# hanquansanren/DvD

Hardware: NVIDIA B200
Metric: dewarped docs/sec (sampling+unwarp) (higher is better)
Workload: dtype bf16x3 (split 16-bit operand pairs, 3 tcgen05 passes per k-step - 2 in the decoder q|k|v GEMMs and the pyramid convs -, fp32 accumulate: fp32-accurate)

## Files before the change

### dvd_b200/_lib.py

```python
from __future__ import annotations

import ctypes as C
import os

_HERE = os.path.dirname(os.path.abspath(__file__))
LIB_PATH = os.environ.get("DVD_LIB", os.path.join(_HERE, "libdvd_b200.so"))

PREC_FP32 = 0
PREC_BF16 = 1
PREC_BF16X3 = 2
TABLE_ROW = 384 + 2304 + 3072

_vp = C.c_void_p


class Mat(C.Structure):
    _fields_ = [("f32", _vp), ("bf16", _vp), ("bf16_lo", _vp), ("n", C.c_int32), ("k", C.c_int32)]


class DecLayer(C.Structure):
    _fields_ = [("n1_w", _vp), ("n1_b", _vp), ("qkv", Mat), ("fc", Mat), ("n2_w", _vp), ("n2_b", _vp),
                ("conv1", Mat), ("bn1_scale", _vp), ("bn1_shift", _vp), ("dw_w", _vp), ("bn2_scale", _vp),
                ("bn2_shift", _vp), ("conv2", Mat), ("bn3_scale", _vp), ("bn3_shift", _vp),
                ("qkv_ln", Mat), ("qkv_colsum", _vp), ("qkv_cvec", _vp), ("conv1_ln", Mat), ("conv1_colsum", _vp), ("conv1_cvec", _vp)]


class Weights(C.Structure):
    _fields_ = [("pos", _vp), ("pyr", Mat * 7), ("pyr_b", _vp * 7), ("emb", Mat * 5), ("emb_b", _vp * 5),
                ("t_mlp0", Mat), ("t_mlp2", Mat), ("t_mlp0_b", _vp), ("t_mlp2_b", _vp),
                ("blk_ada", Mat), ("blk_ada_b", _vp), ("xattn_in", Mat), ("xattn_in_b", _vp),
                ("xattn_out", Mat), ("xattn_out_b", _vp), ("blk_qkv", Mat), ("blk_qkv_b", _vp),
                ("blk_proj", Mat), ("blk_proj_b", _vp), ("blk_fc1", Mat), ("blk_fc1_b", _vp),
                ("blk_fc2", Mat), ("blk_fc2_b", _vp), ("dec_hpe", _vp), ("dec_wpe", _vp),
                ("h_scale0", Mat), ("h_scale2", Mat), ("w_scale0", Mat), ("w_scale2", Mat),
                ("h_scale0_b", _vp), ("h_scale2_b", _vp), ("w_scale0_b", _vp), ("w_scale2_b", _vp),
                ("dec", DecLayer * 6), ("dec_ln_w", _vp), ("dec_ln_b", _vp), ("fin", Mat), ("fin_b", _vp),
                ("fin_ada", Mat), ("fin_ada_b", _vp), ("pyr_h", Mat * 7)]


class UnwarpDoc(C.Structure):
    _fields_ = [("photo", _vp), ("out", _vp), ("H", C.c_int32), ("W", C.c_int32)]


_i, _f, _sz = C.c_int, C.c_float, C.c_size_t
_WP = C.POINTER(Weights)
_FP = C.POINTER(C.c_float)
SIGNATURES = {
    "dvd_version": (_i, []),
    "dvd_last_error": (C.c_char_p, []),
    "dvd_check_device": (_i, []),
    "dvd_unwarp_f32": (_i, [_vp, _vp, _vp, _i, _i, _i, _i, _i, _i, _f, _vp]),
    "dvd_unwarp_u8": (_i, [_vp, _vp, _vp, _i, _i, _i, _i, _i, _i, _f, _vp]),
    "dvd_unwarp_f32_u8": (_i, [_vp, _vp, _vp, _i, _i, _i, _i, _i, _i, _f, _vp]),
    "dvd_unwarp_table_bytes": (_sz, [_i]),
    "dvd_unwarp_u8_plan": (_i, [C.POINTER(UnwarpDoc), _i, _i, _i, _i, _f, _vp, _sz, C.POINTER(C.c_longlong)]),
    "dvd_unwarp_u8_mixed": (_i, [_vp, _i, _vp, _vp]),
    "dvd_grid_sample_f32": (_i, [_vp, _vp, _vp, _i, _i, _i, _i, _i, _i, _vp]),
    "dvd_fullres_grid_f32": (_i, [_vp, _vp, _i, _i, _i, _i, _i, _f, _vp]),
    "dvd_workspace_bytes": (_sz, [_i, _i, _i]),
    "dvd_tables_init": (_i, [_WP, _FP, _i, _vp, _vp]),
    "dvd_static_forward": (_i, [_WP, _vp, _sz, _i, _i, _i, _vp, _vp, _vp, _vp, _vp]),
    "dvd_denoise_step": (_i, [_WP, _vp, _sz, _i, _i, _i, _vp, _vp, _vp, _i, _vp, _f, _f, _vp, _vp, _vp]),
    "dvd_hyp_mean_clamp": (_i, [_vp, _vp, _i, _i, _vp]),
    "dvd_sample": (_i, [_WP, _vp, _sz, _i, _i, _i, _vp, _vp, _vp, _FP, _FP, _FP, _i, _vp, _vp, _vp]),
    "dvd_workspace_feat": (_vp, [_vp, _i, _i, _i]),
    "dvd_workspace_tensor": (_vp, [_vp, _i, _i, _i, C.c_char_p, C.POINTER(C.c_longlong)]),
    "dvd_test_gemm": (_i, [_vp, _vp, _vp, _vp, _i, _i, _i, _i, _vp, _sz, _vp]),
    "dvd_test_attention": (_i, [_vp, _vp, _vp, _vp, _i, _i, _i, _i, _f, _i, _vp, _sz, _vp]),
    "dvd_gemm_bf16": (_i, [_vp, _vp, _i, _vp, _vp, _i, _vp, _vp, _vp, _i, _i, _i, _vp]),
    "dvd_gemm_tune": (_i, [_vp, _vp, _i, _vp, _vp, _i, _vp, _vp, _vp, _i, _vp, _vp, _vp, _vp, _i, _i, _i, _vp]),
    "dvd_debug_stop_after": (_i, [_i]),
    "dvd_profile_begin": (_i, []),
    "dvd_profile_end": (_i, [C.POINTER(C.c_double), C.POINTER(C.c_double), C.POINTER(C.c_longlong), C.POINTER(C.c_double)]),
    "dvd_launch_count": (C.c_longlong, [_i]),
}

_lib = None


def lib() -> C.CDLL:
    global _lib
    if _lib is None:
        if not os.path.exists(LIB_PATH):
            raise RuntimeError(f"{LIB_PATH} not found: the CUDA extension has not been built "
                               "(run `python -m dvd_b200.build`). dvd_b200 has no CPU fallback.")
        l = C.CDLL(LIB_PATH)
        for name, (res, args) in SIGNATURES.items():
            fn = getattr(l, name)
            fn.restype = res
            fn.argtypes = args
        _lib = l
    return _lib


def check(rc: int, what: str = ""):
    if rc != 0:
        msg = lib().dvd_last_error().decode(errors="replace")
        raise RuntimeError(f"libdvd_b200 {what} failed (code {rc}): {msg}")


def ptr(t):
    return None if t is None else _vp(t.data_ptr())


def stream_ptr():
    import torch
    return _vp(torch.cuda.current_stream().cuda_stream)
```

### dvd_b200/csrc/api.cu

```cuda
#include <stdarg.h>
#include <string.h>
#include <stdlib.h>
#include "gemm_simt.cuh"
#include "gemm_tc.cuh"
#include "misc.cuh"

namespace dvd {

static thread_local char g_err[512] = "";
static thread_local long long g_launches = 0;

void set_error(const char* fmt, ...) {
  va_list ap;
  va_start(ap, fmt);
  vsnprintf(g_err, sizeof(g_err), fmt, ap);
  va_end(ap);
}
int cuda_fail(cudaError_t e, const char* what) {
  set_error("CUDA error %d (%s) at %s", (int)e, cudaGetErrorString(e), what);
  return (int)e;
}
void count_launch(int n) { g_launches += n; }
bool pdl_enabled(int kind) {
  static int mask = -1;
// ... 18 lines not shown
extern "C" const char* dvd_last_error(void) { return g_err; }
extern "C" long long dvd_launch_count(int reset) {
  long long v = g_launches;
  if (reset) g_launches = 0;
  return v;
}
extern "C" int dvd_check_device(void) {
  int dev = 0;
  DVD_CUDA(cudaGetDevice(&dev));
  cudaDeviceProp p;
  DVD_CUDA(cudaGetDeviceProperties(&p, dev));
  if (p.major != 10) {
    set_error("device %d is sm_%d%d; libdvd_b200 is built for sm_100a only", dev, p.major, p.minor);
    return DVD_E_ARCH;
  }
  return 0;
}

extern "C" int dvd_test_gemm(const float* A, const float* W, const float* bias, float* C, int M, int N, int K, int precision,
                             void* scratch, size_t scratch_bytes, void* stream) {
  cudaStream_t st = (cudaStream_t)stream;
  DVD_REQUIRE(A && W && C, "test_gemm: null");
  Epilogue e; e.bias = bias; e.out = C; e.ldc = N;
  if (precision == DVD_PREC_FP32) {
    GemmParams p = linear_params(A, K, W, M, N, K);
    p.e = e;
    return gemm_f32(p, A_DIRECT, B_NK, 1, st);
  }
  const bool a16 = precision == 3;
  const bool x3 = precision == DVD_PREC_BF16X3 || a16;
  auto al = [](size_t b) { return (b + 255) & ~size_t(255); };
  const size_t a_b = al((size_t)M * K * 2), w_b = al((size_t)N * K * 2);
  const size_t ops = (x3 ? 2 : 1) * (a_b + w_b);
  DVD_REQUIRE(scratch && scratch_bytes >= ops, "test_gemm: scratch needs %zu bytes", ops);
  char* base = (char*)scratch;
  TcMat a, w;
  a.hi = (__nv_bfloat16*)base; w.hi = (__nv_bfloat16*)(base + a_b); a.ld = K; w.ld = K;
  int rc;
  if (x3) {
    a.lo = (__nv_bfloat16*)(base + a_b + w_b); w.lo = (__nv_bfloat16*)(base + 2 * a_b + w_b);
    if (a16) { rc = f32_to_f16(A, (void*)a.hi, (long long)M * K, st); a.lo = nullptr; a.f16 = true; }
    else rc = f32_split_bf16(A, (__nv_bfloat16*)a.hi, (__nv_bfloat16*)a.lo, (long long)M * K, st);
    if (rc) return rc;
    rc = a16 ? f32_split_f16(W, (void*)w.hi, (void*)w.lo, (long long)N * K, st)
             : f32_split_bf16(W, (__nv_bfloat16*)w.hi, (__nv_bfloat16*)w.lo, (long long)N * K, st);
    if (rc) return rc;
  } else {
    rc = f32_to_bf16(A, (__nv_bfloat16*)a.hi, (long long)M * K, st); if (rc) return rc;
    rc = f32_to_bf16(W, (__nv_bfloat16*)w.hi, (long long)N * K, st); if (rc) return rc;
  }
  return gemm_tc(a, w, M, N, K, e, st);
}

extern "C" int dvd_test_attention(const float* q, const float* k, const float* v, float* o, int batch, int heads, int T, int d,
                                  float scale, int precision, void* scratch, size_t scratch_bytes, void* stream) {
  cudaStream_t st = (cudaStream_t)stream;
  DVD_REQUIRE(q && k && v && o && scratch, "test_attention: null");
  const int ld = heads * d;
  if (precision == DVD_PREC_FP32) {
    size_t per = (size_t)heads * T * T;
    DVD_REQUIRE(scratch_bytes >= per * batch * 4, "test_attention: scratch needs %zu bytes", per * batch * 4);
    float* S = (float*)scratch;
    GemmParams p;
    p.A = q; p.lda = ld; p.sAn = (long long)T * ld; p.sAh = d;
    p.B = k; p.ldb = ld; p.sBn = (long long)T * ld; p.sBh = d;
    p.M = T; p.N = T; p.K = d; p.heads = heads; p.alpha = scale;
    p.e.out = S; p.e.ldc = T; p.sCn = (long long)per; p.sCh = (long long)T * T;
    int rc = gemm_f32(p, A_DIRECT, B_NK, batch * heads, st); if (rc) return rc;
    rc = softmax_rows(S, (long long)batch * heads * T, T, st); if (rc) return rc;
    GemmParams g;
    g.A = S; g.lda = T; g.sAn = (long long)per; g.sAh = (long long)T * T;
    g.B = v; g.ldb = ld; g.sBn = (long long)T * ld; g.sBh = d;
    g.M = T; g.N = d; g.K = T; g.heads = heads;
    g.e.out = o; g.e.ldc = ld; g.sCn = (long long)T * ld; g.sCh = d;
    return gemm_f32(g, A_DIRECT, B_KN, batch * heads, st);
  }
  const bool x3 = precision == DVD_PREC_BF16X3;
  size_t n = (size_t)batch * T * ld;
  DVD_REQUIRE(scratch_bytes >= n * 2 * 6, "test_attention: scratch needs %zu bytes", n * 12);
  __nv_bfloat16* q16 = (__nv_bfloat16*)scratch; __nv_bfloat16* k16 = q16 + n; __nv_bfloat16* v16 = k16 + n; __nv_bfloat16* o16 = v16 + n;
  __nv_bfloat16* vt16 = o16 + n; __nv_bfloat16* olo = vt16 + n;
  int rc;
  if (x3) {
    rc = f32_to_f16(q, q16, n, st); if (rc) return rc;
    rc = f32_to_f16(k, k16, n, st); if (rc) return rc;
    rc = f32_to_f16(v, v16, n, st); if (rc) return rc;
  } else {
    rc = f32_to_bf16(q, q16, n, st); if (rc) return rc;
    rc = f32_to_bf16(k, k16, n, st); if (rc) return rc;
    rc = f32_to_bf16(v, v16, n, st); if (rc) return rc;
  }
  rc = transpose_v16(v16, ld, vt16, batch, T, ld, st); if (rc) return rc;
  rc = attention_tc(q16, ld, k16, ld, vt16, o16, x3 ? olo : nullptr, ld, batch, heads, T, d, scale, 1, x3 ? 1 : 0, st); if (rc) return rc;
  return pair_to_f32(o16, x3 ? olo : nullptr, o, n, st);
}

extern "C" int dvd_gemm_bf16(const void* A16, const void* A16_lo, int lda, const void* W16, const void* W16_lo, int ldw, const float* bias,
                             void* out16, float* out32, int M, int N, int K, void* stream) {
  Epilogue e; e.bias = bias; e.out_bf16 = (__nv_bfloat16*)out16; e.ldc_bf16 = N; e.out = out32; e.ldc = N;
  TcMat a, w;
  a.hi = (const __nv_bfloat16*)A16; a.lo = (const __nv_bfloat16*)A16_lo; a.ld = lda;
  a.f16 = !A16_lo && W16_lo;
  w.hi = (const __nv_bfloat16*)W16; w.lo = (const __nv_bfloat16*)W16_lo; w.ld = ldw;
  return gemm_tc(a, w, M, N, K, e, (cudaStream_t)stream);
}

// ... 13 lines not shown
```

### dvd_b200/csrc/misc.cu

```cuda
#include "misc.cuh"
#include "tc_epilogue.cuh"
#include <algorithm>

namespace dvd {

template <int NV>
__global__ void __launch_bounds__(256) k_layernorm(const float* __restrict__ in, int ldin, float* __restrict__ out, int ldo,
                                                   __nv_bfloat16* __restrict__ out16, __nv_bfloat16* __restrict__ out16_lo, int ldo16,
                                                   int rows, float eps, const float* __restrict__ w, const float* __restrict__ b,
                                                   const float* __restrict__ msh, const float* __restrict__ msc) {
  pdl_trigger();
  pdl_wait();
  const int row = blockIdx.x * 8 + (threadIdx.x >> 5), lane = threadIdx.x & 31;
  if (row >= rows) return;
  constexpr int C = 128 * NV;
  const float4* x4 = reinterpret_cast<const float4*>(in + (size_t)row * ldin);
  float4 v[NV];
  float s = 0.f;
#pragma unroll
  for (int i = 0; i < NV; ++i) { v[i] = __ldg(x4 + lane + 32 * i); s += (v[i].x + v[i].y) + (v[i].z + v[i].w); }
  const float mean = warp_sum(s) * (1.0f / C);
  float q = 0.f;
#pragma unroll
  for (int i = 0; i < NV; ++i) {
// ... 510 lines not shown
  float s1 = 0.f, s2 = 0.f;
#pragma unroll
  for (int i = 0; i < 12; ++i) {
    const int c = lane + 32 * i;
    float4 x = xr[c];
    const float4 a = __ldg(hs + (size_t)n * C4 + c), b = __ldg(ws + (size_t)n * C4 + c);
    const float4 hp = __ldg(hpe + (size_t)(tok >> 5) * C4 + c), wp = __ldg(wpe + (size_t)(tok & 31) * C4 + c);
    x.x = (x.x + a.x * hp.x) + b.x * wp.x; x.y = (x.y + a.y * hp.y) + b.y * wp.y;
    x.z = (x.z + a.z * hp.z) + b.z * wp.z; x.w = (x.w + a.w * hp.w) + b.w * wp.w;
    xr[c] = x;
    *reinterpret_cast<uint2*>(x16 + ((size_t)row * C4 + c) * 4) = make_uint2(pack_f16x2(x.x, x.y), pack_f16x2(x.z, x.w));
    s1 += (x.x + x.y) + (x.z + x.w);
    s2 += (x.x * x.x + x.y * x.y) + (x.z * x.z + x.w * x.w);
  }
  s1 = warp_sum(s1); s2 = warp_sum(s2);
  float2* sr = reinterpret_cast<float2*>(stats) + (size_t)row * chunks;
  for (int k = lane; k < chunks; k += 32) sr[k] = k == 0 ? make_float2(s1, s2) : make_float2(0.f, 0.f);
}
int posenc_add_ln(float* X, const float* hs, const float* ws, const float* hpe, const float* wpe, int N, int C, __nv_bfloat16* x16,
                  float* stats, int chunks, cudaStream_t st) {
  DVD_REQUIRE(X && hs && ws && hpe && wpe && x16 && stats && C == 1536 && chunks == C / 32, "posenc_add_ln: bad args");
  const int rows = N * 1024;
  DVD_CUDA(launch_pdl(16, k_posenc_ln, dim3(cdiv(rows, 8)), dim3(256), (size_t)0, st, X, (const float4*)hs, (const float4*)ws, (const float4*)hpe,
                      (const float4*)wpe, x16, stats, chunks, rows));
  DVD_LAUNCH_CHECK("k_posenc_ln");
  return 0;
}

__global__ void __launch_bounds__(256) k_dwconv(const float4* __restrict__ in, const float4* __restrict__ w9, const float4* __restrict__ sc,
                                                const float4* __restrict__ sh, float* __restrict__ out, __nv_bfloat16* __restrict__ out16,
                                                int C4, size_t total) {
  size_t i = (size_t)blockIdx.x * blockDim.x + threadIdx.x;
  if (i >= total) return;
  int c = i % C4; size_t row = i / C4;
  int tok = row % 1024; size_t n = row / 1024;
  int y = tok / 32, x = tok % 32;
  float4 acc = make_float4(0.f, 0.f, 0.f, 0.f);
#pragma unroll
  for (int ky = 0; ky < 3; ++ky) {
    int yy = y + ky - 1;
    if (yy < 0 || yy >= 32) continue;
#pragma unroll
    for (int kx = 0; kx < 3; ++kx) {
      int xx = x + kx - 1;
      if (xx < 0 || xx >= 32) continue;
      float4 v = __ldg(in + (n * 1024 + yy * 32 + xx) * C4 + c), ww = __ldg(w9 + (size_t)(ky * 3 + kx) * C4 + c);
      acc.x = fmaf(v.x, ww.x, acc.x); acc.y = fmaf(v.y, ww.y, acc.y); acc.z = fmaf(v.z, ww.z, acc.z); acc.w = fmaf(v.w, ww.w, acc.w);
    }
  }
  float4 s = __ldg(sc + c), t = __ldg(sh + c);
  float r0 = fmaxf(acc.x * s.x + t.x, 0.f), r1 = fmaxf(acc.y * s.y + t.y, 0.f), r2 = fmaxf(acc.z * s.z + t.z, 0.f), r3 = fmaxf(acc.w * s.w + t.w, 0.f);
  store4(out, Out16{out16, nullptr}, i * 4, r0, r1, r2, r3);
}
template <int RS, int NW>
__global__ void __launch_bounds__(32 * NW) k_dwconv_bf16(const uint4* __restrict__ in, const uint4* __restrict__ in_lo, const float* __restrict__ w9,
                                                     const float* __restrict__ sc, const float* __restrict__ sh, uint4* __restrict__ out,
                                                     uint4* __restrict__ out_lo, int C8) {
  __shared__ __align__(16) float s_w[9][256];
  __shared__ __align__(16) float s_sc[256], s_sh[256];
  pdl_trigger();
  const int lane = threadIdx.x & 31, warp = threadIdx.x >> 5;
  const int c8 = blockIdx.x * 32 + lane;
  const int x = blockIdx.y * NW + warp;
  const int strips = 32 / RS;
  const size_t n = blockIdx.z / strips;
  const int y0 = (blockIdx.z % strips) * RS;
  const int C = C8 * 8, cb = blockIdx.x * 256;
  for (int e = threadIdx.x; e < 9 * 256; e += 32 * NW) s_w[e >> 8][e & 255] = (cb + (e & 255) < C) ? __ldg(w9 + (size_t)(e >> 8) * C + cb + (e & 255)) : 0.f;
  for (int e = threadIdx.x; e < 256; e += 32 * NW) {
    s_sc[e] = (cb + e < C) ? __ldg(sc + cb + e) : 0.f;
    s_sh[e] = (cb + e < C) ? __ldg(sh + cb + e) : 0.f;
  }
  __syncthreads();
  pdl_wait();
  if (c8 >= C8) return;
  float acc[RS][8];
#pragma unroll
  for (int o = 0; o < RS; ++o)
#pragma unroll
    for (int k = 0; k < 8; ++k) acc[o][k] = 0.f;
#pragma unroll 1
  for (int kx = 0; kx < 3; ++kx) {
    const int xx = x + kx - 1;
    if (xx < 0 || xx >= 32) continue;
    float w[3][8];
#pragma unroll
    for (int ky = 0; ky < 3; ++ky) {
      const float4 w0 = *reinterpret_cast<const float4*>(&s_w[ky * 3 + kx][lane * 8]);
      const float4 w1 = *reinterpret_cast<const float4*>(&s_w[ky * 3 + kx][lane * 8 + 4]);
      w[ky][0] = w0.x; w[ky][1] = w0.y; w[ky][2] = w0.z; w[ky][3] = w0.w; w[ky][4] = w1.x; w[ky][5] = w1.y; w[ky][6] = w1.z; w[ky][7] = w1.w;
    }
#pragma unroll
    for (int r = -1; r <= RS; ++r) {
      const int yy = y0 + r;
      if (yy < 0 || yy >= 32) continue;
      const uint4 v = __ldg(in + (n * 1024 + yy * 32 + xx) * C8 + c8);
      const __nv_bfloat162* h = reinterpret_cast<const __nv_bfloat162*>(&v);
      float f[8] = {__low2float(h[0]), __high2float(h[0]), __low2float(h[1]), __high2float(h[1]),
                    __low2float(h[2]), __high2float(h[2]), __low2float(h[3]), __high2float(h[3])};
      if (in_lo) {
        const uint4 vl = __ldg(in_lo + (n * 1024 + yy * 32 + xx) * C8 + c8);
        const __nv_bfloat162* hl = reinterpret_cast<const __nv_bfloat162*>(&vl);
#pragma unroll
        for (int k = 0; k < 4; ++k) { f[2 * k] += __low2float(hl[k]); f[2 * k + 1] += __high2float(hl[k]); }
      }
#pragma unroll
      for (int ky = 0; ky < 3; ++ky) {
        const int o = r + 1 - ky;
        if (o < 0 || o >= RS) continue;
#pragma unroll
        for (int k = 0; k < 8; ++k) acc[o][k] = fmaf(f[k], w[ky][k], acc[o][k]);
      }
    }
  }
  const float4 s0 = *reinterpret_cast<const float4*>(&s_sc[lane * 8]), s1 = *reinterpret_cast<const float4*>(&s_sc[lane * 8 + 4]);
  const float4 t0 = *reinterpret_cast<const float4*>(&s_sh[lane * 8]), t1 = *reinterpret_cast<const float4*>(&s_sh[lane * 8 + 4]);
#pragma unroll
  for (int o = 0; o < RS; ++o) {
    const float r8[8] = {fmaxf(acc[o][0] * s0.x + t0.x, 0.f), fmaxf(acc[o][1] * s0.y + t0.y, 0.f), fmaxf(acc[o][2] * s0.z + t0.z, 0.f),
                         fmaxf(acc[o][3] * s0.w + t0.w, 0.f), fmaxf(acc[o][4] * s1.x + t1.x, 0.f), fmaxf(acc[o][5] * s1.y + t1.y, 0.f),
                         fmaxf(acc[o][6] * s1.z + t1.z, 0.f), fmaxf(acc[o][7] * s1.w + t1.w, 0.f)};
    uint4 ov, ol;
    split_bf16x2(r8[0], r8[1], ov.x, ol.x); split_bf16x2(r8[2], r8[3], ov.y, ol.y);
    split_bf16x2(r8[4], r8[5], ov.z, ol.z); split_bf16x2(r8[6], r8[7], ov.w, ol.w);
    out[(n * 1024 + (size_t)(y0 + o) * 32 + x) * C8 + c8] = ov;
    if (out_lo) out_lo[(n * 1024 + (size_t)(y0 + o) * 32 + x) * C8 + c8] = ol;
  }
}
int dwconv3x3_bn_relu_bf16(const __nv_bfloat16* in, const __nv_bfloat16* in_lo, const float* w9c, const float* scale, const float* shift,
                           __nv_bfloat16* out, __nv_bfloat16* out_lo, int N, int C, cudaStream_t st) {
  DVD_REQUIRE(in && w9c && scale && shift && out && C % 8 == 0, "dwconv_bf16: bad args");
  constexpr int RS = 4, NW = 4;
  DVD_REQUIRE((long long)N * (32 / RS) <= 65535, "dwconv_bf16: batch too large for the grid");
  DVD_CUDA(launch_pdl(8, k_dwconv_bf16<RS, NW>, dim3(cdiv(C / 8, 32), 32 / NW, N * (32 / RS)), dim3(32 * NW), (size_t)0, st, (const uint4*)in, (const uint4*)in_lo, w9c, scale,
                      shift, (uint4*)out, (uint4*)out_lo, C / 8));
  DVD_LAUNCH_CHECK("k_dwconv_bf16");
  return 0;
}

int dwconv3x3_bn_relu(const float* in, const float* w9c, const float* scale, const float* shift, float* out, __nv_bfloat16* out16,
                      int N, int C, cudaStream_t st) {
  DVD_REQUIRE(in && w9c && scale && shift && (out || out16) && C % 4 == 0, "dwconv: bad args");
  size_t total = (size_t)N * 1024 * (C / 4);
  k_dwconv<<<cdiv(total, 256), 256, 0, st>>>((const float4*)in, (const float4*)w9c, (const float4*)scale, (const float4*)shift, out, out16,
                                             C / 4, total);
  DVD_LAUNCH_CHECK("k_dwconv");
  return 0;
}

__global__ void __launch_bounds__(256) k_final(const float* __restrict__ X, const float* __restrict__ lw, const float* __restrict__ lb,
                                               const float* __restrict__ shift, const float* __restrict__ scale,
                                               const float* __restrict__ W8, const float* __restrict__ b8,
                                               const float* __restrict__ init_flow, const float* __restrict__ x_t, float a, float b,
                                               float* __restrict__ pred, float* __restrict__ x_prev, int rows) {
  pdl_trigger();
  pdl_wait();
  const int row = blockIdx.x * 8 + (threadIdx.x >> 5), lane = threadIdx.x & 31;
  if (row >= rows) return;
  constexpr int NV = 12, C = 1536;
  const float4* x4 = reinterpret_cast<const float4*>(X + (size_t)row * C);
  float v[NV][4];
  float s = 0.f;
#pragma unroll
  for (int i = 0; i < NV; ++i) {
    float4 t = __ldg(x4 + lane + 32 * i);
    v[i][0] = t.x; v[i][1] = t.y; v[i][2] = t.z; v[i][3] = t.w;
    s += (t.x + t.y) + (t.z + t.w);
  }
  float mean = warp_sum(s) * (1.0f / C), q = 0.f;
#pragma unroll
  for (int i = 0; i < NV; ++i)
#pragma unroll
    for (int j = 0; j < 4; ++j) { float d = v[i][j] - mean; q += d * d; }
  float rstd = 1.0f / sqrtf(warp_sum(q) * (1.0f / C) + 1e-5f);
  s = 0.f;
#pragma unroll
  for (int i = 0; i < NV; ++i) {
    const int c0 = (lane + 32 * i) * 4;
    float4 ww = __ldg(reinterpret_cast<const float4*>(lw + c0)), bb = __ldg(reinterpret_cast<const float4*>(lb + c0));
    v[i][0] = (v[i][0] - mean) * rstd * ww.x + bb.x; v[i][1] = (v[i][1] - mean) * rstd * ww.y + bb.y;
    v[i][2] = (v[i][2] - mean) * rstd * ww.z + bb.z; v[i][3] = (v[i][3] - mean) * rstd * ww.w + bb.w;
    s += (v[i][0] + v[i][1]) + (v[i][2] + v[i][3]);
  }
  mean = warp_sum(s) * (1.0f / C); q = 0.f;
#pragma unroll
  for (int i = 0; i < NV; ++i)
#pragma unroll
    for (int j = 0; j < 4; ++j) { float d = v[i][j] - mean; q += d * d; }
  rstd = 1.0f / sqrtf(warp_sum(q) * (1.0f / C) + 1e-6f);
// ... 124 lines not shown
```

### include/dvd_b200.h

```cpp
#ifndef DVD_B200_H
#define DVD_B200_H

#include <stddef.h>
#include <stdint.h>

#ifdef __cplusplus
extern "C" {
#endif

#define DVD_ABI_VERSION 5

#if defined(__GNUC__)
#define DVD_API __attribute__((visibility("default")))
#else
#define DVD_API
#endif

#define DVD_E_BADARG   (-1)
#define DVD_E_ARCH     (-2)
#define DVD_E_WORKSPACE (-3)
#define DVD_E_NOTMA    (-4)

#define DVD_PREC_FP32  0
#define DVD_PREC_BF16  1
// ... 53 lines not shown
DVD_API const char* dvd_last_error(void);
DVD_API int         dvd_check_device(void);

DVD_API int dvd_unwarp_f32(const float* photo, const float* map, float* out, int B, int C, int H, int W,
                   int mh, int mw, float affine, void* stream);
DVD_API int dvd_unwarp_u8(const uint8_t* photo, const float* map, uint8_t* out, int B, int C, int H, int W,
                  int mh, int mw, float affine, void* stream);
DVD_API int dvd_unwarp_f32_u8(const float* photo, const float* map, uint8_t* out, int B, int C, int H, int W,
                      int mh, int mw, float affine, void* stream);
typedef struct dvd_unwarp_doc {
  const uint8_t* photo;
  uint8_t* out;
  int32_t H, W;
} dvd_unwarp_doc_t;
DVD_API size_t dvd_unwarp_table_bytes(int max_docs);
DVD_API int dvd_unwarp_u8_plan(const dvd_unwarp_doc_t* docs_host, int n_docs, int C, int mh, int mw, float affine,
                               void* table_host, size_t table_bytes, long long* total_tiles);
DVD_API int dvd_unwarp_u8_mixed(const void* table, int C, const float* map, void* stream);
DVD_API int dvd_grid_sample_f32(const float* img, const float* grid, float* out, int B, int C, int H, int W,
                        int Ho, int Wo, void* stream);
DVD_API int dvd_fullres_grid_f32(const float* map, float* grid, int B, int H, int W, int mh, int mw,
                         float affine, void* stream);

DVD_API size_t dvd_workspace_bytes(int docs, int n_hyp, int precision);

DVD_API int dvd_tables_init(const dvd_weights_t* w, const float* t_values_host, int n_steps, float* tables,
                    void* stream);

DVD_API int dvd_static_forward(const dvd_weights_t* w, void* workspace, size_t workspace_bytes, int docs,
                       int n_hyp, int precision, const float* y512, const float* mask_cat,
                       const float* mask_y512, const float* line_msk, void* stream);

DVD_API int dvd_denoise_step(const dvd_weights_t* w, void* workspace, size_t workspace_bytes, int docs,
                     int n_hyp, int precision, const float* x_t, const float* init_flow,
                     const float* init_feat, int feat_is_init, const float* table_row,
                     float ddim_a, float ddim_b, float* pred_x0, float* x_prev, void* stream);

DVD_API int dvd_hyp_mean_clamp(const float* pred_x0, float* out, int docs, int n_hyp, void* stream);

DVD_API int dvd_sample(const dvd_weights_t* w, void* workspace, size_t workspace_bytes, int docs, int n_hyp,
               int precision, const float* x_T, const float* init_flow0, const float* tables,
               const float* t_scaled_host, const float* ddim_a_host, const float* ddim_b_host,
               int S, const float* init_feat0, float* map_out, void* stream);

DVD_API const float* dvd_workspace_feat(void* workspace, int docs, int n_hyp, int precision);

DVD_API const float* dvd_workspace_tensor(void* workspace, int docs, int n_hyp, int precision, const char* name,
                                          long long* numel);

DVD_API int dvd_debug_stop_after(int stage);

DVD_API int dvd_test_gemm(const float* A, const float* W, const float* bias, float* C, int M, int N, int K,
                  int precision, void* scratch, size_t scratch_bytes, void* stream);
DVD_API int dvd_test_attention(const float* q, const float* k, const float* v, float* o, int batch, int heads,
                       int T, int d, float scale, int precision, void* scratch, size_t scratch_bytes,
                       void* stream);
DVD_API int dvd_gemm_bf16(const void* A16, const void* A16_lo, int lda, const void* W16, const void* W16_lo, int ldw,
                          const float* bias, void* out16, float* out32, int M, int N, int K, void* stream);
DVD_API int dvd_gemm_tune(const void* A16, const void* A16_lo, int lda, const void* W16, const void* W16_lo, int ldw,
                          const float* bias, const float* scale, const float* shift, int relu, void* out16, void* out16_lo,
                          float* out32, const float* resid, int M, int N, int K, void* stream);
DVD_API int dvd_profile_begin(void);
DVD_API int dvd_profile_end(double* ms, double* flops, long long* launches, double* executed_flops);
DVD_API long long dvd_launch_count(int reset);

#ifdef __cplusplus
}
#endif
#endif
```

Measured before the change: 223.5.

## Stage depthwise-conv input bands in shared memory and use packed FMA

Rewrites the 3x3 depthwise conv+BN+ReLU kernel used in the decoder. Each block now loads a 64-channel by (8+2)-row band of the 32x32 image once into shared memory as fp32, merging the hi/lo bf16 halves at load time. Previously every output re-read its neighbours from global memory, repeating the hi+lo decode for each tap. The inner loop now uses packed float2 FMAs, and weight loads are issued before the PDL wait to overlap with the previous kernel. In exchange it needs about 80KB of dynamic shared memory per block and C must be a multiple of 64. A test entry point is also added.

```diff
diff --git a/dvd_b200/_lib.py b/dvd_b200/_lib.py
--- a/dvd_b200/_lib.py
+++ b/dvd_b200/_lib.py
@@ -66,6 +66,7 @@
     "dvd_workspace_feat": (_vp, [_vp, _i, _i, _i]),
     "dvd_workspace_tensor": (_vp, [_vp, _i, _i, _i, C.c_char_p, C.POINTER(C.c_longlong)]),
     "dvd_test_gemm": (_i, [_vp, _vp, _vp, _vp, _i, _i, _i, _i, _vp, _sz, _vp]),
+    "dvd_test_dwconv": (_i, [_vp, _vp, _vp, _vp, _vp, _vp, _vp, _i, _i, _vp]),
     "dvd_test_attention": (_i, [_vp, _vp, _vp, _vp, _i, _i, _i, _i, _f, _i, _vp, _sz, _vp]),
     "dvd_gemm_bf16": (_i, [_vp, _vp, _i, _vp, _vp, _i, _vp, _vp, _vp, _i, _i, _i, _vp]),
     "dvd_gemm_tune": (_i, [_vp, _vp, _i, _vp, _vp, _i, _vp, _vp, _vp, _i, _vp, _vp, _vp, _vp, _i, _i, _i, _vp]),
diff --git a/dvd_b200/csrc/api.cu b/dvd_b200/csrc/api.cu
--- a/dvd_b200/csrc/api.cu
+++ b/dvd_b200/csrc/api.cu
@@ -94,6 +94,12 @@
   return gemm_tc(a, w, M, N, K, e, st);
 }
 
+extern "C" int dvd_test_dwconv(const void* in, const void* in_lo, const float* w9c, const float* scale, const float* shift, void* out,
+                               void* out_lo, int N, int C, void* stream) {
+  return dwconv3x3_bn_relu_bf16((const __nv_bfloat16*)in, (const __nv_bfloat16*)in_lo, w9c, scale, shift, (__nv_bfloat16*)out,
+                                (__nv_bfloat16*)out_lo, N, C, (cudaStream_t)stream);
+}
+
 extern "C" int dvd_test_attention(const float* q, const float* k, const float* v, float* o, int batch, int heads, int T, int d,
                                   float scale, int precision, void* scratch, size_t scratch_bytes, void* stream) {
   cudaStream_t st = (cudaStream_t)stream;
diff --git a/dvd_b200/csrc/misc.cu b/dvd_b200/csrc/misc.cu
--- a/dvd_b200/csrc/misc.cu
+++ b/dvd_b200/csrc/misc.cu
@@ -586,89 +586,115 @@
   float r0 = fmaxf(acc.x * s.x + t.x, 0.f), r1 = fmaxf(acc.y * s.y + t.y, 0.f), r2 = fmaxf(acc.z * s.z + t.z, 0.f), r3 = fmaxf(acc.w * s.w + t.w, 0.f);
   store4(out, Out16{out16, nullptr}, i * 4, r0, r1, r2, r3);
 }
-template <int RS, int NW>
-__global__ void __launch_bounds__(32 * NW) k_dwconv_bf16(const uint4* __restrict__ in, const uint4* __restrict__ in_lo, const float* __restrict__ w9,
-                                                     const float* __restrict__ sc, const float* __restrict__ sh, uint4* __restrict__ out,
-                                                     uint4* __restrict__ out_lo, int C8) {
-  __shared__ __align__(16) float s_w[9][256];
-  __shared__ __align__(16) float s_sc[256], s_sh[256];
-  pdl_trigger();
-  const int lane = threadIdx.x & 31, warp = threadIdx.x >> 5;
-  const int c8 = blockIdx.x * 32 + lane;
-  const int x = blockIdx.y * NW + warp;
-  const int strips = 32 / RS;
-  const size_t n = blockIdx.z / strips;
-  const int y0 = (blockIdx.z % strips) * RS;
-  const int C = C8 * 8, cb = blockIdx.x * 256;
-  for (int e = threadIdx.x; e < 9 * 256; e += 32 * NW) s_w[e >> 8][e & 255] = (cb + (e & 255) < C) ? __ldg(w9 + (size_t)(e >> 8) * C + cb + (e & 255)) : 0.f;
-  for (int e = threadIdx.x; e < 256; e += 32 * NW) {
-    s_sc[e] = (cb + e < C) ? __ldg(sc + cb + e) : 0.f;
-    s_sh[e] = (cb + e < C) ? __ldg(sh + cb + e) : 0.f;
+constexpr int kDwCh = 64;
+template <int BAND>
+__global__ void __launch_bounds__(256, 2) k_dwconv_tile(const uint4* __restrict__ in, const uint4* __restrict__ in_lo,
+                                                        const float4* __restrict__ w9, const float4* __restrict__ sc,
+                                                        const float4* __restrict__ sh, uint4* __restrict__ out,
+                                                        uint4* __restrict__ out_lo, int C) {
+  constexpr int ROWS = BAND + 2;
+  extern __shared__ __align__(16) float4 s_x[];
+  __shared__ __align__(16) float4 s_w[9 * 16 + 2 * 16];
+  pdl_trigger();
+  const int tid = threadIdx.x, C4 = C / 4, C8 = C / 8;
+  const int c0 = blockIdx.x * kDwCh, y0 = blockIdx.y * BAND;
+  const size_t n = blockIdx.z;
+  float4 wv = make_float4(0.f, 0.f, 0.f, 0.f);
+  if (tid < 9 * 16) wv = __ldg(w9 + (size_t)(tid >> 4) * C4 + c0 / 4 + (tid & 15));
+  else if (tid < 10 * 16) wv = __ldg(sc + c0 / 4 + tid - 9 * 16);
+  else if (tid < 11 * 16) wv = __ldg(sh + c0 / 4 + tid - 10 * 16);
+  pdl_wait();
+  {
+    const int col = tid >> 3, q = tid & 7;
+    uint4 vh[ROWS], vl[ROWS];
+#pragma unroll
+    for (int i = 0; i < ROWS; ++i) {
+      const int yy = y0 - 1 + i;
+      if (yy >= 0 && yy < 32) {
+        const size_t gi = (n * 1024 + yy * 32 + col) * C8 + c0 / 8 + q;
+        vh[i] = __ldg(in + gi);
+        if (in_lo) vl[i] = __ldg(in_lo + gi);
+      }
+    }
+    if (tid < 11 * 16) s_w[tid] = wv;
+#pragma unroll
+    for (int i = 0; i < ROWS; ++i) {
+      const int yy = y0 - 1 + i;
+      if (yy < 0 || yy >= 32) continue;
+      const __nv_bfloat162* h = reinterpret_cast<const __nv_bfloat162*>(&vh[i]);
+      float2 f[4];
+#pragma unroll
+      for (int k = 0; k < 4; ++k) f[k] = __bfloat1622float2(h[k]);
+      if (in_lo) {
+        const __nv_bfloat162* hl = reinterpret_cast<const __nv_bfloat162*>(&vl[i]);
+#pragma unroll
+        for (int k = 0; k < 4; ++k) f[k] = __fadd2_rn(f[k], __bfloat1622float2(hl[k]));
+      }
+      s_x[(i * 32 + col) * 16 + q] = make_float4(f[0].x, f[0].y, f[1].x, f[1].y);
+      s_x[(i * 32 + col) * 16 + 8 + q] = make_float4(f[2].x, f[2].y, f[3].x, f[3].y);
+    }
   }
   __syncthreads();
-  pdl_wait();
-  if (c8 >= C8) return;
-  float acc[RS][8];
-#pragma unroll
-  for (int o = 0; o < RS; ++o)
-#pragma unroll
-    for (int k = 0; k < 8; ++k) acc[o][k] = 0.f;
+  const int lane = tid & 31, g = lane & 7;
+  const int x = (tid >> 5) * 4 + (lane >> 3);
+  float2 acc[BAND][4];
+#pragma unroll
+  for (int o = 0; o < BAND; ++o)
+#pragma unroll
+    for (int k = 0; k < 4; ++k) acc[o][k] = make_float2(0.f, 0.f);
 #pragma unroll 1
   for (int kx = 0; kx < 3; ++kx) {
     const int xx = x + kx - 1;
     if (xx < 0 || xx >= 32) continue;
-    float w[3][8];
+    float2 w[3][4];
 #pragma unroll
     for (int ky = 0; ky < 3; ++ky) {
-      const float4 w0 = *reinterpret_cast<const float4*>(&s_w[ky * 3 + kx][lane * 8]);
-      const float4 w1 = *reinterpret_cast<const float4*>(&s_w[ky * 3 + kx][lane * 8 + 4]);
-      w[ky][0] = w0.x; w[ky][1] = w0.y; w[ky][2] = w0.z; w[ky][3] = w0.w; w[ky][4] = w1.x; w[ky][5] = w1.y; w[ky][6] = w1.z; w[ky][7] = w1.w;
-    }
-#pragma unroll
-    for (int r = -1; r <= RS; ++r) {
-      const int yy = y0 + r;
+      const float4 w0 = s_w[(ky * 3 + kx) * 16 + 2 * g], w1 = s_w[(ky * 3 + kx) * 16 + 2 * g + 1];
+      w[ky][0] = make_float2(w0.x, w0.y); w[ky][1] = make_float2(w0.z, w0.w); w[ky][2] = make_float2(w1.x, w1.y); w[ky][3] = make_float2(w1.z, w1.w);
+    }
+#pragma unroll
+    for (int i = 0; i < ROWS; ++i) {
+      const int yy = y0 - 1 + i;
       if (yy < 0 || yy >= 32) continue;
-      const uint4 v = __ldg(in + (n * 1024 + yy * 32 + xx) * C8 + c8);
-      const __nv_bfloat162* h = reinterpret_cast<const __nv_bfloat162*>(&v);
-      float f[8] = {__low2float(h[0]), __high2float(h[0]), __low2float(h[1]), __high2float(h[1]),
-                    __low2float(h[2]), __high2float(h[2]), __low2float(h[3]), __high2float(h[3])};
-      if (in_lo) {
-        const uint4 vl = __ldg(in_lo + (n * 1024 + yy * 32 + xx) * C8 + c8);
-        const __nv_bfloat162* hl = reinterpret_cast<const __nv_bfloat162*>(&vl);
-#pragma unroll
-        for (int k = 0; k < 4; ++k) { f[2 * k] += __low2float(hl[k]); f[2 * k + 1] += __high2float(hl[k]); }
+      const float4 a = s_x[(i * 32 + xx) * 16 + g], b = s_x[(i * 32 + xx) * 16 + 8 + g];
+      const float2 f[4] = {make_float2(a.x, a.y), make_float2(a.z, a.w), make_float2(b.x, b.y), make_float2(b.z, b.w)};
+#pragma unroll
+      for (int ky = 0; ky < 3; ++ky) {
+        const int o = i - ky;
+        if (o < 0 || o >= BAND) continue;
+#pragma unroll
+        for (int k = 0; k < 4; ++k) acc[o][k] = __ffma2_rn(f[k], w[ky][k], acc[o][k]);
       }
-#pragma unroll
-      for (int ky = 0; ky < 3; ++ky) {
-        const int o = r + 1 - ky;
-        if (o < 0 || o >= RS) continue;
-#pragma unroll
-        for (int k = 0; k < 8; ++k) acc[o][k] = fmaf(f[k], w[ky][k], acc[o][k]);
-      }
-    }
-  }
-  const float4 s0 = *reinterpret_cast<const float4*>(&s_sc[lane * 8]), s1 = *reinterpret_cast<const float4*>(&s_sc[lane * 8 + 4]);
-  const float4 t0 = *reinterpret_cast<const float4*>(&s_sh[lane * 8]), t1 = *reinterpret_cast<const float4*>(&s_sh[lane * 8 + 4]);
-#pragma unroll
-  for (int o = 0; o < RS; ++o) {
-    const float r8[8] = {fmaxf(acc[o][0] * s0.x + t0.x, 0.f), fmaxf(acc[o][1] * s0.y + t0.y, 0.f), fmaxf(acc[o][2] * s0.z + t0.z, 0.f),
-                         fmaxf(acc[o][3] * s0.w + t0.w, 0.f), fmaxf(acc[o][4] * s1.x + t1.x, 0.f), fmaxf(acc[o][5] * s1.y + t1.y, 0.f),
-                         fmaxf(acc[o][6] * s1.z + t1.z, 0.f), fmaxf(acc[o][7] * s1.w + t1.w, 0.f)};
+    }
+  }
+  const float4 s0 = s_w[9 * 16 + 2 * g], s1 = s_w[9 * 16 + 2 * g + 1];
+  const float4 t0 = s_w[10 * 16 + 2 * g], t1 = s_w[10 * 16 + 2 * g + 1];
+#pragma unroll
+  for (int o = 0; o < BAND; ++o) {
+    const float r8[8] = {fmaxf(acc[o][0].x * s0.x + t0.x, 0.f), fmaxf(acc[o][0].y * s0.y + t0.y, 0.f), fmaxf(acc[o][1].x * s0.z + t0.z, 0.f),
+                         fmaxf(acc[o][1].y * s0.w + t0.w, 0.f), fmaxf(acc[o][2].x * s1.x + t1.x, 0.f), fmaxf(acc[o][2].y * s1.y + t1.y, 0.f),
+                         fmaxf(acc[o][3].x * s1.z + t1.z, 0.f), fmaxf(acc[o][3].y * s1.w + t1.w, 0.f)};
     uint4 ov, ol;
     split_bf16x2(r8[0], r8[1], ov.x, ol.x); split_bf16x2(r8[2], r8[3], ov.y, ol.y);
     split_bf16x2(r8[4], r8[5], ov.z, ol.z); split_bf16x2(r8[6], r8[7], ov.w, ol.w);
-    out[(n * 1024 + (size_t)(y0 + o) * 32 + x) * C8 + c8] = ov;
-    if (out_lo) out_lo[(n * 1024 + (size_t)(y0 + o) * 32 + x) * C8 + c8] = ol;
+    const size_t oi = (n * 1024 + (size_t)(y0 + o) * 32 + x) * C8 + c0 / 8 + g;
+    out[oi] = ov;
+    if (out_lo) out_lo[oi] = ol;
   }
 }
 int dwconv3x3_bn_relu_bf16(const __nv_bfloat16* in, const __nv_bfloat16* in_lo, const float* w9c, const float* scale, const float* shift,
                            __nv_bfloat16* out, __nv_bfloat16* out_lo, int N, int C, cudaStream_t st) {
-  DVD_REQUIRE(in && w9c && scale && shift && out && C % 8 == 0, "dwconv_bf16: bad args");
-  constexpr int RS = 4, NW = 4;
-  DVD_REQUIRE((long long)N * (32 / RS) <= 65535, "dwconv_bf16: batch too large for the grid");
-  DVD_CUDA(launch_pdl(8, k_dwconv_bf16<RS, NW>, dim3(cdiv(C / 8, 32), 32 / NW, N * (32 / RS)), dim3(32 * NW), (size_t)0, st, (const uint4*)in, (const uint4*)in_lo, w9c, scale,
-                      shift, (uint4*)out, (uint4*)out_lo, C / 8));
-  DVD_LAUNCH_CHECK("k_dwconv_bf16");
+  DVD_REQUIRE(in && w9c && scale && shift && out && N > 0 && C > 0, "dwconv_bf16: bad args");
+  DVD_REQUIRE(C % kDwCh == 0, "dwconv_bf16: C must be a multiple of %d (got %d)", kDwCh, C);
+  DVD_REQUIRE(N <= 65535, "dwconv_bf16: batch too large for the grid");
+  DVD_REQUIRE(((uintptr_t)in | (uintptr_t)in_lo | (uintptr_t)w9c | (uintptr_t)scale | (uintptr_t)shift | (uintptr_t)out | (uintptr_t)out_lo) % 16 == 0,
+              "dwconv_bf16: pointers must be 16-byte aligned");
+  constexpr int BAND = 8;
+  constexpr size_t smem = (size_t)(BAND + 2) * 32 * kDwCh * 4;
+  DVD_SET_MAX_SMEM(k_dwconv_tile<BAND>, smem);
+  DVD_CUDA(launch_pdl(8, k_dwconv_tile<BAND>, dim3(C / kDwCh, 32 / BAND, N), dim3(256), smem, st, (const uint4*)in, (const uint4*)in_lo,
+                      (const float4*)w9c, (const float4*)scale, (const float4*)shift, (uint4*)out, (uint4*)out_lo, C));
+  DVD_LAUNCH_CHECK("k_dwconv_tile");
   return 0;
 }
 
diff --git a/include/dvd_b200.h b/include/dvd_b200.h
--- a/include/dvd_b200.h
+++ b/include/dvd_b200.h
@@ -129,6 +129,8 @@
 
 DVD_API int dvd_test_gemm(const float* A, const float* W, const float* bias, float* C, int M, int N, int K,
                   int precision, void* scratch, size_t scratch_bytes, void* stream);
+DVD_API int dvd_test_dwconv(const void* in, const void* in_lo, const float* w9c, const float* scale, const float* shift,
+                            void* out, void* out_lo, int N, int C, void* stream);
 DVD_API int dvd_test_attention(const float* q, const float* k, const float* v, float* o, int batch, int heads,
                        int T, int d, float scale, int precision, void* scratch, size_t scratch_bytes,
                        void* stream);
```

Result: faster. 230.0, median of 6 (+2.9%).

## Rewrite depthwise 3x3 conv as persistent smem-tiled kernel with paired FMA

Applied to the files above, without the earlier changes.

Replaces the register-strip depthwise conv (one warp per column, global loads per tap) with a persistent kernel that stages a 10-row band of a 64-channel slice (hi and lo halves) into shared memory via cp.async. Each thread then computes a 4x4 spatial output block over 4 channels using packed float2 FMAs, reusing each loaded pixel across neighbouring outputs. The grid is sized from occupancy. The goal is to cut redundant global reads and instruction count. In exchange it requires C to be a multiple of 64 and 16-byte-aligned pointers, and it adds a test entry point.

```diff
diff --git a/dvd_b200/_lib.py b/dvd_b200/_lib.py
--- a/dvd_b200/_lib.py
+++ b/dvd_b200/_lib.py
@@ -66,6 +66,7 @@
     "dvd_workspace_feat": (_vp, [_vp, _i, _i, _i]),
     "dvd_workspace_tensor": (_vp, [_vp, _i, _i, _i, C.c_char_p, C.POINTER(C.c_longlong)]),
     "dvd_test_gemm": (_i, [_vp, _vp, _vp, _vp, _i, _i, _i, _i, _vp, _sz, _vp]),
+    "dvd_test_dwconv": (_i, [_vp, _vp, _vp, _vp, _vp, _vp, _vp, _i, _i, _vp]),
     "dvd_test_attention": (_i, [_vp, _vp, _vp, _vp, _i, _i, _i, _i, _f, _i, _vp, _sz, _vp]),
     "dvd_gemm_bf16": (_i, [_vp, _vp, _i, _vp, _vp, _i, _vp, _vp, _vp, _i, _i, _i, _vp]),
     "dvd_gemm_tune": (_i, [_vp, _vp, _i, _vp, _vp, _i, _vp, _vp, _vp, _i, _vp, _vp, _vp, _vp, _i, _i, _i, _vp]),
diff --git a/dvd_b200/csrc/api.cu b/dvd_b200/csrc/api.cu
--- a/dvd_b200/csrc/api.cu
+++ b/dvd_b200/csrc/api.cu
@@ -94,6 +94,12 @@
   return gemm_tc(a, w, M, N, K, e, st);
 }
 
+extern "C" int dvd_test_dwconv(const void* in, const void* in_lo, const float* w9c, const float* scale, const float* shift, void* out,
+                               void* out_lo, int N, int C, void* stream) {
+  return dwconv3x3_bn_relu_bf16((const __nv_bfloat16*)in, (const __nv_bfloat16*)in_lo, w9c, scale, shift, (__nv_bfloat16*)out,
+                                (__nv_bfloat16*)out_lo, N, C, (cudaStream_t)stream);
+}
+
 extern "C" int dvd_test_attention(const float* q, const float* k, const float* v, float* o, int batch, int heads, int T, int d,
                                   float scale, int precision, void* scratch, size_t scratch_bytes, void* stream) {
   cudaStream_t st = (cudaStream_t)stream;
diff --git a/dvd_b200/csrc/misc.cu b/dvd_b200/csrc/misc.cu
--- a/dvd_b200/csrc/misc.cu
+++ b/dvd_b200/csrc/misc.cu
@@ -586,88 +586,125 @@
   float r0 = fmaxf(acc.x * s.x + t.x, 0.f), r1 = fmaxf(acc.y * s.y + t.y, 0.f), r2 = fmaxf(acc.z * s.z + t.z, 0.f), r3 = fmaxf(acc.w * s.w + t.w, 0.f);
   store4(out, Out16{out16, nullptr}, i * 4, r0, r1, r2, r3);
 }
-template <int RS, int NW>
-__global__ void __launch_bounds__(32 * NW) k_dwconv_bf16(const uint4* __restrict__ in, const uint4* __restrict__ in_lo, const float* __restrict__ w9,
-                                                     const float* __restrict__ sc, const float* __restrict__ sh, uint4* __restrict__ out,
-                                                     uint4* __restrict__ out_lo, int C8) {
-  __shared__ __align__(16) float s_w[9][256];
-  __shared__ __align__(16) float s_sc[256], s_sh[256];
-  pdl_trigger();
-  const int lane = threadIdx.x & 31, warp = threadIdx.x >> 5;
-  const int c8 = blockIdx.x * 32 + lane;
-  const int x = blockIdx.y * NW + warp;
-  const int strips = 32 / RS;
-  const size_t n = blockIdx.z / strips;
-  const int y0 = (blockIdx.z % strips) * RS;
-  const int C = C8 * 8, cb = blockIdx.x * 256;
-  for (int e = threadIdx.x; e < 9 * 256; e += 32 * NW) s_w[e >> 8][e & 255] = (cb + (e & 255) < C) ? __ldg(w9 + (size_t)(e >> 8) * C + cb + (e & 255)) : 0.f;
-  for (int e = threadIdx.x; e < 256; e += 32 * NW) {
-    s_sc[e] = (cb + e < C) ? __ldg(sc + cb + e) : 0.f;
-    s_sh[e] = (cb + e < C) ? __ldg(sh + cb + e) : 0.f;
-  }
-  __syncthreads();
-  pdl_wait();
-  if (c8 >= C8) return;
-  float acc[RS][8];
-#pragma unroll
-  for (int o = 0; o < RS; ++o)
-#pragma unroll
-    for (int k = 0; k < 8; ++k) acc[o][k] = 0.f;
-#pragma unroll 1
-  for (int kx = 0; kx < 3; ++kx) {
-    const int xx = x + kx - 1;
-    if (xx < 0 || xx >= 32) continue;
-    float w[3][8];
-#pragma unroll
-    for (int ky = 0; ky < 3; ++ky) {
-      const float4 w0 = *reinterpret_cast<const float4*>(&s_w[ky * 3 + kx][lane * 8]);
-      const float4 w1 = *reinterpret_cast<const float4*>(&s_w[ky * 3 + kx][lane * 8 + 4]);
-      w[ky][0] = w0.x; w[ky][1] = w0.y; w[ky][2] = w0.z; w[ky][3] = w0.w; w[ky][4] = w1.x; w[ky][5] = w1.y; w[ky][6] = w1.z; w[ky][7] = w1.w;
-    }
-#pragma unroll
-    for (int r = -1; r <= RS; ++r) {
-      const int yy = y0 + r;
-      if (yy < 0 || yy >= 32) continue;
-      const uint4 v = __ldg(in + (n * 1024 + yy * 32 + xx) * C8 + c8);
-      const __nv_bfloat162* h = reinterpret_cast<const __nv_bfloat162*>(&v);
-      float f[8] = {__low2float(h[0]), __high2float(h[0]), __low2float(h[1]), __high2float(h[1]),
-                    __low2float(h[2]), __high2float(h[2]), __low2float(h[3]), __high2float(h[3])};
-      if (in_lo) {
-        const uint4 vl = __ldg(in_lo + (n * 1024 + yy * 32 + xx) * C8 + c8);
-        const __nv_bfloat162* hl = reinterpret_cast<const __nv_bfloat162*>(&vl);
-#pragma unroll
-        for (int k = 0; k < 4; ++k) { f[2 * k] += __low2float(hl[k]); f[2 * k + 1] += __high2float(hl[k]); }
+constexpr int kDwBand = 8, kDwSlice = 64, kDwThreads = 256;
+constexpr size_t kDwTileBytes = (size_t)(kDwBand + 2) * 32 * kDwSlice * 4;
+
+__device__ __forceinline__ void cp_async16(void* smem, const void* gmem) {
+  asm volatile("cp.async.cg.shared.global [%0], [%1], 16;" ::"r"((uint32_t)__cvta_generic_to_shared(smem)), "l"(gmem) : "memory");
+}
+__device__ __forceinline__ void bf16x4_to_f32(uint2 v, float2& a, float2& b) {
+  const __nv_bfloat162* h = reinterpret_cast<const __nv_bfloat162*>(&v);
+  a = make_float2(__low2float(h[0]), __high2float(h[0]));
+  b = make_float2(__low2float(h[1]), __high2float(h[1]));
+}
+
+__global__ void __launch_bounds__(kDwThreads, 2) k_dwconv_bf16(const uint4* __restrict__ in, const uint4* __restrict__ in_lo,
+                                                              const float* __restrict__ w9, const float* __restrict__ sc,
+                                                              const float* __restrict__ sh, uint2* __restrict__ out,
+                                                              uint2* __restrict__ out_lo, int C, int units) {
+  extern __shared__ uint4 s_tile[];
+  pdl_trigger();
+  const int t = threadIdx.x, s = t & 15, j = (t >> 4) & 1, q = t >> 5;
+  const int C8 = C / 8, slices = C / kDwSlice;
+  const bool pair = in_lo != nullptr;
+  for (int u = blockIdx.x; u < units; u += gridDim.x) {
+    const int cs = u % slices, y0 = (u / slices) % (32 / kDwBand) * kDwBand;
+    const size_t n = u / (slices * (32 / kDwBand));
+    float4 w[9];
+#pragma unroll
+    for (int k = 0; k < 9; ++k) w[k] = __ldg(reinterpret_cast<const float4*>(w9 + (size_t)k * C + cs * kDwSlice) + s);
+    const float4 bs = __ldg(reinterpret_cast<const float4*>(sc + cs * kDwSlice) + s);
+    const float4 bt = __ldg(reinterpret_cast<const float4*>(sh + cs * kDwSlice) + s);
+    if (u == (int)blockIdx.x) pdl_wait();
+    else __syncthreads();
+    {
+      const int g = t & 7, x = t >> 3;
+#pragma unroll
+      for (int r = 0; r < kDwBand + 2; ++r) {
+        const int yy = y0 - 1 + r;
+        if (yy < 0 || yy >= 32) continue;
+        const size_t src = (n * 1024 + yy * 32 + x) * C8 + cs * 8 + g;
+        uint4* dst = s_tile + (r * 32 + x) * 16;
+        cp_async16(dst + g, in + src);
+        if (pair) cp_async16(dst + 8 + g, in_lo + src);
       }
-#pragma unroll
-      for (int ky = 0; ky < 3; ++ky) {
-        const int o = r + 1 - ky;
-        if (o < 0 || o >= RS) continue;
-#pragma unroll
-        for (int k = 0; k < 8; ++k) acc[o][k] = fmaf(f[k], w[ky][k], acc[o][k]);
+      asm volatile("cp.async.wait_all;" ::: "memory");
+    }
+    __syncthreads();
+    const uint2* tile = reinterpret_cast<const uint2*>(s_tile);
+    float2 acc[4][4][2];
+#pragma unroll
+    for (int k = 0; k < 4; ++k)
+#pragma unroll
+      for (int o = 0; o < 4; ++o) acc[k][o][0] = acc[k][o][1] = make_float2(0.f, 0.f);
+#pragma unroll
+    for (int i = 0; i < 6; ++i) {
+      const int xx = 4 * q - 1 + i;
+      if (xx >= 0 && xx < 32) {
+#pragma unroll
+        for (int rr = 0; rr < 6; ++rr) {
+          const int yy = y0 + 4 * j - 1 + rr;
+          if (yy < 0 || yy >= 32) continue;
+          const uint2* px = tile + ((4 * j + rr) * 32 + xx) * 32;
+          float2 f0, f1;
+          bf16x4_to_f32(px[s], f0, f1);
+          if (pair) {
+            float2 l0, l1;
+            bf16x4_to_f32(px[16 + s], l0, l1);
+            f0 = __fadd2_rn(f0, l0); f1 = __fadd2_rn(f1, l1);
+          }
+#pragma unroll
+          for (int ky = 0; ky < 3; ++ky) {
+            const int o = rr - ky;
+            if (o < 0 || o >= 4) continue;
+#pragma unroll
+            for (int k = 0; k < 4; ++k) {
+              const int kx = i - k;
+              if (kx < 0 || kx > 2) continue;
+              const float4 ww = w[ky * 3 + kx];
+              acc[k][o][0] = __ffma2_rn(f0, make_float2(ww.x, ww.y), acc[k][o][0]);
+              acc[k][o][1] = __ffma2_rn(f1, make_float2(ww.z, ww.w), acc[k][o][1]);
+            }
+          }
+        }
       }
-    }
-  }
-  const float4 s0 = *reinterpret_cast<const float4*>(&s_sc[lane * 8]), s1 = *reinterpret_cast<const float4*>(&s_sc[lane * 8 + 4]);
-  const float4 t0 = *reinterpret_cast<const float4*>(&s_sh[lane * 8]), t1 = *reinterpret_cast<const float4*>(&s_sh[lane * 8 + 4]);
-#pragma unroll
-  for (int o = 0; o < RS; ++o) {
-    const float r8[8] = {fmaxf(acc[o][0] * s0.x + t0.x, 0.f), fmaxf(acc[o][1] * s0.y + t0.y, 0.f), fmaxf(acc[o][2] * s0.z + t0.z, 0.f),
-                         fmaxf(acc[o][3] * s0.w + t0.w, 0.f), fmaxf(acc[o][4] * s1.x + t1.x, 0.f), fmaxf(acc[o][5] * s1.y + t1.y, 0.f),
-                         fmaxf(acc[o][6] * s1.z + t1.z, 0.f), fmaxf(acc[o][7] * s1.w + t1.w, 0.f)};
-    uint4 ov, ol;
-    split_bf16x2(r8[0], r8[1], ov.x, ol.x); split_bf16x2(r8[2], r8[3], ov.y, ol.y);
-    split_bf16x2(r8[4], r8[5], ov.z, ol.z); split_bf16x2(r8[6], r8[7], ov.w, ol.w);
-    out[(n * 1024 + (size_t)(y0 + o) * 32 + x) * C8 + c8] = ov;
-    if (out_lo) out_lo[(n * 1024 + (size_t)(y0 + o) * 32 + x) * C8 + c8] = ol;
+      if (i >= 2) {
+        const int k = i - 2;
+#pragma unroll
+        for (int o = 0; o < 4; ++o) {
+          const float r0 = fmaxf(fmaf(acc[k][o][0].x, bs.x, bt.x), 0.f), r1 = fmaxf(fmaf(acc[k][o][0].y, bs.y, bt.y), 0.f);
+          const float r2 = fmaxf(fmaf(acc[k][o][1].x, bs.z, bt.z), 0.f), r3 = fmaxf(fmaf(acc[k][o][1].y, bs.w, bt.w), 0.f);
+          uint2 ov, ol;
+          split_bf16x2(r0, r1, ov.x, ol.x); split_bf16x2(r2, r3, ov.y, ol.y);
+          const size_t o4 = (n * 1024 + (size_t)(y0 + 4 * j + o) * 32 + 4 * q + k) * (C / 4) + cs * (kDwSlice / 4) + s;
+          out[o4] = ov;
+          if (out_lo) out_lo[o4] = ol;
+        }
+      }
+    }
   }
 }
 int dwconv3x3_bn_relu_bf16(const __nv_bfloat16* in, const __nv_bfloat16* in_lo, const float* w9c, const float* scale, const float* shift,
                            __nv_bfloat16* out, __nv_bfloat16* out_lo, int N, int C, cudaStream_t st) {
-  DVD_REQUIRE(in && w9c && scale && shift && out && C % 8 == 0, "dwconv_bf16: bad args");
-  constexpr int RS = 4, NW = 4;
-  DVD_REQUIRE((long long)N * (32 / RS) <= 65535, "dwconv_bf16: batch too large for the grid");
-  DVD_CUDA(launch_pdl(8, k_dwconv_bf16<RS, NW>, dim3(cdiv(C / 8, 32), 32 / NW, N * (32 / RS)), dim3(32 * NW), (size_t)0, st, (const uint4*)in, (const uint4*)in_lo, w9c, scale,
-                      shift, (uint4*)out, (uint4*)out_lo, C / 8));
+  DVD_REQUIRE(in && w9c && scale && shift && out && N >= 1 && C >= kDwSlice && C % kDwSlice == 0, "dwconv_bf16: bad args (N=%d, C=%d)", N, C);
+  const long long units = (long long)N * (32 / kDwBand) * (C / kDwSlice);
+  DVD_REQUIRE(units <= 0x7fffffff, "dwconv_bf16: batch too large");
+  auto misaligned = [](const void* p) { return ((uintptr_t)p & 15) != 0; };
+  DVD_REQUIRE(!misaligned(in) && !misaligned(in_lo) && !misaligned(w9c) && !misaligned(scale) && !misaligned(shift) && !misaligned(out) &&
+                  !misaligned(out_lo), "dwconv_bf16: every pointer must be 16-byte aligned");
+  int dev = 0, n_sm = 0;
+  DVD_CUDA(cudaGetDevice(&dev));
+  DVD_REQUIRE(dev < 64, "dwconv_bf16: device %d", dev);
+  DVD_CUDA(cudaDeviceGetAttribute(&n_sm, cudaDevAttrMultiProcessorCount, dev));
+  DVD_SET_MAX_SMEM(k_dwconv_bf16, kDwTileBytes);
+  static int per_sm[64] = {};
+  if (!per_sm[dev]) {
+    DVD_CUDA(cudaOccupancyMaxActiveBlocksPerMultiprocessor(&per_sm[dev], k_dwconv_bf16, kDwThreads, kDwTileBytes));
+    DVD_REQUIRE(per_sm[dev] >= 1, "dwconv_bf16: kernel does not fit an SM");
+  }
+  const int grid = (int)std::min<long long>(units, (long long)n_sm * per_sm[dev]);
+  DVD_CUDA(launch_pdl(8, k_dwconv_bf16, dim3(grid), dim3(kDwThreads), kDwTileBytes, st, (const uint4*)in, (const uint4*)in_lo, w9c, scale,
+                      shift, (uint2*)out, (uint2*)out_lo, C, (int)units));
   DVD_LAUNCH_CHECK("k_dwconv_bf16");
   return 0;
 }
diff --git a/include/dvd_b200.h b/include/dvd_b200.h
--- a/include/dvd_b200.h
+++ b/include/dvd_b200.h
@@ -132,6 +132,8 @@
 DVD_API int dvd_test_attention(const float* q, const float* k, const float* v, float* o, int batch, int heads,
                        int T, int d, float scale, int precision, void* scratch, size_t scratch_bytes,
                        void* stream);
+DVD_API int dvd_test_dwconv(const void* in, const void* in_lo, const float* w9c, const float* scale, const float* shift, void* out,
+                            void* out_lo, int N, int C, void* stream);
 DVD_API int dvd_gemm_bf16(const void* A16, const void* A16_lo, int lda, const void* W16, const void* W16_lo, int ldw,
                           const float* bias, void* out16, float* out32, int M, int N, int K, void* stream);
 DVD_API int dvd_gemm_tune(const void* A16, const void* A16_lo, int lda, const void* W16, const void* W16_lo, int ldw,
```

Measured after the change: 220.5 before, 227.7 after (median of 6 runs). 3.3% higher.
